# bcgsc/goldrush

Measured on AMD Instinct MI355X. Metric: reads/s through GoldRush-Path (hash + miBF query), higher is better.
Workload: dtype u64

## Files before the change

### goldrush_amd/csrc/grp_batch.inc

```

namespace {

constexpr uint32_t BATCH_MAX_INS = 1u << 17;
constexpr uint32_t BATCH_MAX_BLOCKS = 256;
constexpr uint64_t BATCH_MAX_REC = 1ull << 26;
constexpr unsigned long long BATCH_LOW26 = (1ull << 26) - 1ull;

struct DevBatch
{
  uint32_t epoch = 0;
  uint32_t* bits = nullptr;
  uint64_t cap_mask = 0;
  uint32_t* counters = nullptr;
  uint32_t* chained = nullptr;
  const uint32_t* ins = nullptr;
  uint32_t n_ins = 0, block_tiles = 0;
  uint32_t n_rec = 0;
  unsigned long long* rec_key = nullptr;
  unsigned long long* rec_loc = nullptr;
  unsigned long long* rec_old = nullptr;
  uint32_t* rec_chain = nullptr;
  uint32_t* ovf_next = nullptr;
  uint32_t* ovf_jb = nullptr;
  uint32_t ovf_cap = 0;
// ... 1 lines not shown
  uint32_t* log_head = nullptr;
  uint32_t* log_old = nullptr;
  uint32_t* log_writer = nullptr;
  uint32_t* log_next = nullptr;
  uint32_t* log_slot = nullptr;
  uint64_t log_mask = 0;
  uint32_t log_cap = 0;
  uint32_t first_read = 0;
};

__device__ inline uint32_t
batch_block_id(const DevBatch& b, uint32_t jb)
{
  const uint32_t j = jb >> 8, blk = jb & 255u;
  const uint32_t* e = b.ins + (size_t)j * 6;
  return e[3] + (blk * b.block_tiles + e[4]) / b.block_tiles;
}

__device__ inline uint32_t
wave_counter_take(uint32_t* ctr)
{
  const unsigned long long here = __ballot(1);
  const uint32_t lane = threadIdx.x & 63u;
  const uint32_t leader = (uint32_t)__ffsll((long long)here) - 1u;
  uint32_t base = 0;
  if (lane == leader) {
    base = atomicAdd(ctr, (uint32_t)__popcll(here));
  }
  base = __shfl(base, (int)leader, 64);
  return base + (uint32_t)__popcll(here & ((1ull << lane) - 1ull));
}

__device__ inline uint32_t
batch_unit_jb(const DevBatch& b, uint32_t unit, uint32_t parts)
{
  uint32_t lo = 0, hi = b.n_ins;
  while (hi - lo > 1) {
    const uint32_t mid = (lo + hi) >> 1;
    if (b.ins[(size_t)mid * 6 + 5] <= unit) {
      lo = mid;
    } else {
      hi = mid;
    }
  }
  const uint32_t tj = (unit - b.ins[(size_t)lo * 6 + 5]) / parts;
  return (lo << 8) | (tj / b.block_tiles);
}

template<int H, int WT>
__global__ void __launch_bounds__(THREADS)
k_batch_collect(DevFilter f, DevReads rd, const DevSeeds* __restrict__ sd, uint32_t tile_len, DevBatch b, uint32_t gunit0)
{
  extern __shared__ uint4 smem4[];
  ulonglong2* sTab = reinterpret_cast<ulonglong2*>(smem4);
  const uint32_t hn = frame_seeds<H>(sd);
  uint32_t* sBases = reinterpret_cast<uint32_t*>(sTab + hn * sd->wmax * 4u);

  const uint32_t gunit = gunit0 + blockIdx.x;
  const uint32_t unit = gunit / hn;
  const uint32_t s = gunit - unit * hn;
  const uint32_t parts = gr::geom::tile_parts(frames_per_tile(sd, tile_len));
  const uint32_t jb = batch_unit_jb(b, unit, parts);
  const uint32_t* e = b.ins + (size_t)(jb >> 8) * 6;
  const uint32_t read_idx = e[0], tile_start = e[1];
  const uint32_t u = unit - e[5];
  const uint32_t tj = u / parts, part = u - tj * parts;
  const uint32_t ti = tile_start + tj;
  const uint32_t blk_unit0 = e[5] + (tj / b.block_tiles) * b.block_tiles * parts;
  const uint32_t blk_unit1 = min(blk_unit0 + b.block_tiles * parts, e[5] + (e[2] - e[1]) * parts);
  const uint32_t len = rd.len[read_idx];
  const gr::geom::TileExtent ext = tile_extent(sd, tile_len, len, ti);
  const uint32_t start = ext.start, Lp = ext.Lp, frames = ext.frames;

  load_tab(sTab, sd);
  const uint32_t boff = stage_bases(sBases, rd.packed, rd.word_off[read_idx], len, start, Lp);
  __syncthreads();

  const uint32_t fr = part * THREADS + threadIdx.x;
  const bool live = fr < frames;
  const uint32_t fs = min(min(fr, frames ? frames - 1u : 0u), Lp - sd->span[s]);
  const Probe pr = grp_locate(f, seed_hash_t<WT>(sTab, sd, s, window_at(sBases, boff + fs)));
  uint32_t lr, rel, bit, qid = 0;
  {
    const uint32_t sub = threadIdx.x & 3u, quad_base = (threadIdx.x & 63u) & ~3u;
    const uint4 p0 = f.buckets[quad_bcast64<0>(pr.b) * GRP_UNIT_U4 + sub];
    const uint4 p1 = f.buckets[quad_bcast64<1>(pr.b) * GRP_UNIT_U4 + sub];
    const uint4 p2 = f.buckets[quad_bcast64<2>(pr.b) * GRP_UNIT_U4 + sub];
    const uint4 p3 = f.buckets[quad_bcast64<3>(pr.b) * GRP_UNIT_U4 + sub];
    const QuadAnswer a0 = quad_answer<0>(p0, pr.off, quad_base);
    const QuadAnswer a1 = quad_answer<1>(p1, pr.off, quad_base);
    const QuadAnswer a2 = quad_answer<2>(p2, pr.off, quad_base);
    const QuadAnswer a3 = quad_answer<3>(p3, pr.off, quad_base);
    const QuadAnswer mine = (sub == 0) ? a0 : (sub == 1) ? a1 : (sub == 2) ? a2 : a3;
    lr = mine.lr;
    rel = mine.rel;
    bit = mine.bit;
    qid = mine.id;
  }
  const uint64_t rank = f.super[pr.b >> GRP_SUPER_SHIFT] + rel + lr;
  const bool valid = live && rank < f.pop && bit;
  const uint32_t idx = gunit * THREADS + threadIdx.x;
  const uint64_t home = ((rank + 1) * 0x9E3779B97F4A7C15ULL) >> 20 & b.cap_mask;
  bool claimed = false;
  uint32_t count0 = 0;
  uint32_t* idp = nullptr;
  uint32_t id0 = 0;
  uint32_t why = !live ? 0u : 1u;
  if (valid) {
    unsigned long long* cwp = grp_cw_ptr(f, pr.b, lr, rank);
    idp = (lr < GRP_BUCKET_IDS) ? &reinterpret_cast<uint32_t*>(f.buckets)[grp_id_loc(pr.b, lr)] : nullptr;
    id0 = idp ? qid : 1u;
    unsigned long long cur = (id0 == 0u) ? 0ull : __hip_atomic_load(cwp, __ATOMIC_RELAXED, __HIP_MEMORY_SCOPE_AGENT);
    for (;;) {
      if (grp_claim_epoch(cur) == b.epoch) {
        const uint32_t owner = grp_claim_record(cur);
        const uint32_t owner_unit = owner / (hn * THREADS);
        why = owner + 2u;
        if (owner_unit < blk_unit0 || owner_unit >= blk_unit1) {
          const uint32_t at = wave_counter_take(&b.counters[1]);
          if (at < b.ovf_cap) {
            b.ovf_jb[at] = jb;
            const uint32_t before = atomicExch(&b.rec_chain[owner], at);
            b.ovf_next[at] = before;
            if (before == BATCH_NONE) {
              b.chained[wave_counter_take(&b.counters[0])] = owner;
            }
          }
        }
        break;
      }
      count0 = grp_cnt(cur);
      const unsigned long long prev = atomicCAS(cwp, cur, grp_cnt_with(grp_claim_word(idx, b.epoch, 0u), count0 + 1u));
      if (prev == cur) {
        claimed = true;
        break;
      }
      cur = prev;
    }
  }
  b.rec_key[idx] = claimed ? (((unsigned long long)(rank + 1) << 26) | jb) : (unsigned long long)why;
  if (claimed) {
    const unsigned long long loc = grp_id_loc(pr.b, lr);
    uint32_t* p = idp;
    const uint32_t cur = p ? id0 : grp_ovf_get(f, rank);
    const uint32_t cnt = count0 + 1u;
    const uint32_t id = batch_block_id(b, jb);
    const bool wrote = (uint32_t)(rank ^ (uint64_t)id) % cnt == cnt - 1u;
    if (wrote && cur != 0u) {
      atomicOr(&b.bits[home >> 5], 1u << (home & 31u));
    }
    if (wrote) {
      const uint32_t nv = (cur > 0x80000000u) ? (id | 0x80000000u) : id;
      if (p) {
        *p = nv;
      } else {
        grp_ovf_put(f, rank, nv);
      }
    }
    b.rec_loc[idx] = loc;
    b.rec_old[idx] = ((unsigned long long)(wrote ? 1u : 0u) << 63) | ((unsigned long long)count0 << 32) | cur;
  }
}



__device__ inline uint32_t
batch_next_touch(const DevBatch& b, uint32_t chain, uint32_t own_jb, uint32_t last)
{
  uint32_t best = BATCH_NONE;
  if (last == BATCH_NONE || own_jb > last) {
    best = own_jb;
  }
  for (uint32_t e = chain; e != BATCH_NONE; e = b.ovf_next[e]) {
    const uint32_t jb = b.ovf_jb[e];
    if ((last == BATCH_NONE || jb > last) && jb < best) {
      best = jb;
// ... 689 lines not shown
```

### goldrush_amd/csrc/grp_kernels.inc

```

__device__ inline uint64_t
window_lo(const uint32_t* sBases, uint32_t b)
{
  uint32_t bit = b * 2u;
  uint32_t wi = bit >> 5;
  uint32_t sh = bit & 31u;
  uint64_t lo = (uint64_t)sBases[wi] | ((uint64_t)sBases[wi + 1] << 32);
  uint64_t w = lo >> sh;
  if (sh) {
    w |= (uint64_t)sBases[wi + 2] << (64u - sh);
  }
  return w;
}

struct Win
{
  uint64_t lo;
  const uint32_t* src;
  uint32_t b;
};

__device__ inline Win
window_at(const uint32_t* sBases, uint32_t b)
{
// ... 357 lines not shown
      for (uint32_t q = 1; q < GRP_UNIT_U4; ++q) {
        buckets[b * GRP_UNIT_U4 + q] = make_uint4(0, 0, 0, 0);
      }
    }
    rel += (uint32_t)__popcll(bm[i]);
  }
  ovf = wave_sum(ovf);
  far = wave_sum(far);
  if ((threadIdx.x & 63) == 0 && ovf) {
    atomicAdd(n_ovf, (unsigned long long)ovf);
  }
  if ((threadIdx.x & 63) == 0 && far) {
    atomicAdd(n_ovf + 1, (unsigned long long)far);
  }
}

__global__ void __launch_bounds__(THREADS)
k_far_build(DevFilter f)
{
  for (uint64_t b = (uint64_t)blockIdx.x * THREADS + threadIdx.x; b < f.n_buckets; b += (uint64_t)gridDim.x * THREADS) {
    const uint4 hd = f.buckets[b * GRP_UNIT_U4];
    const uint32_t c = (uint32_t)__popcll(grp_bitmap(hd));
    if (c <= GRP_NEAR_CW) {
      continue;
    }
    const uint64_t base = f.super[b >> GRP_SUPER_SHIFT] + hd.x;
    for (uint32_t lr = GRP_NEAR_CW; lr < c; ++lr) {
      const unsigned long long key = base + lr + 1;
      uint64_t slot = (key * 0x9E3779B97F4A7C15ULL) >> 19 & f.far_mask;
      for (;;) {
        if (f.far[slot].x == 0ull && atomicCAS(&f.far[slot].x, 0ull, key) == 0ull) {
          break;
        }
        slot = (slot + 1) & f.far_mask;
      }
    }
  }
}

__global__ void __launch_bounds__(THREADS)
k_far_reset(ulonglong2* __restrict__ far, uint64_t n)
{
  for (uint64_t i = (uint64_t)blockIdx.x * THREADS + threadIdx.x; i < n; i += (uint64_t)gridDim.x * THREADS) {
    far[i].y = 0ull;
  }
}

__global__ void __launch_bounds__(THREADS)
k_reset_bucket_ids(uint4* __restrict__ buckets, uint64_t n_buckets)
{
  for (uint64_t i = (uint64_t)blockIdx.x * THREADS + threadIdx.x; i < n_buckets * GRP_UNIT_U4; i += (uint64_t)gridDim.x * THREADS) {
    if ((i & (GRP_UNIT_U4 - 1u)) == 0) {
      reinterpret_cast<uint32_t*>(&buckets[i])[3] = 0u;
    } else {
      buckets[i] = make_uint4(0, 0, 0, 0);
    }
  }
}


template<int G>
__device__ inline uint32_t
quad_bcast(uint32_t v)
{
  return (uint32_t)__builtin_amdgcn_mov_dpp((int)v, G * 0x55, 0xF, 0xF, true);
}

template<int G>
__device__ inline uint64_t
quad_bcast64(uint64_t v)
{
  return (uint64_t)quad_bcast<G>((uint32_t)v) | ((uint64_t)quad_bcast<G>((uint32_t)(v >> 32)) << 32);
}

struct QuadAnswer
{
  uint32_t bit;
  uint32_t lr;
  uint32_t id;
  uint32_t rel;
};

template<int G>
__device__ inline QuadAnswer
quad_answer(const uint4& piece, uint32_t off, uint32_t quad_base)
{
  const uint32_t o = quad_bcast<G>(off);
  const uint64_t bm = (uint64_t)quad_bcast<0>(piece.y) | ((uint64_t)quad_bcast<0>(piece.z) << 32);
  QuadAnswer a;
  a.rel = quad_bcast<0>(piece.x);
  a.bit = (uint32_t)((bm >> o) & 1ull);
  a.lr = grp_local_rank(bm, o);
  const uint32_t slot = 3u + min(a.lr, GRP_BUCKET_IDS - 1u);
  const uint32_t comp = slot & 3u;
  const uint32_t word = (comp == 0u) ? piece.x : (comp == 1u) ? piece.y : (comp == 2u) ? piece.z : piece.w;
  a.id = (uint32_t)__builtin_amdgcn_ds_bpermute((int)((quad_base + (slot >> 2)) << 2), (int)word);
  return a;
}


__device__ inline void
hist_add(uint32_t* keys, uint32_t* cnts, uint32_t mask, uint32_t id, uint32_t* sDistinct, uint32_t limit, uint32_t* sOverflow)
{
  if (*reinterpret_cast<volatile uint32_t*>(sDistinct) >= limit) {
    *sOverflow = 1u;
    return;
  }
  uint32_t slot = (id * 2654435761u) & mask;
  for (;;) {
    uint32_t old = atomicCAS(&keys[slot], 0u, id);
    if (old == 0u) {
      atomicAdd(sDistinct, 1u);
    }
    if (old == 0u || old == id) {
      atomicAdd(&cnts[slot], 1u);
      return;
    }
    slot = (slot + 1u) & mask;
  }
}

__device__ inline void
hist_add16(uint32_t* keys, uint32_t* cnt_words, uint32_t cap, uint32_t id, uint32_t* sDistinct, uint32_t limit, uint32_t* sOverflow)
{
  if (*reinterpret_cast<volatile uint32_t*>(sDistinct) >= limit) {
    *sOverflow = 1u;
    return;
  }
  uint32_t slot = __umulhi(id * 2654435761u, cap);
  for (;;) {
    uint32_t old = atomicCAS(&keys[slot], 0u, id);
    if (old == 0u) {
      atomicAdd(sDistinct, 1u);
    }
    if (old == 0u || old == id) {
      atomicAdd(&cnt_words[slot >> 1], 1u << ((slot & 1u) << 4));
      return;
    }
    slot = (slot + 1u == cap) ? 0u : slot + 1u;
  }
}

__device__ inline bool
better(uint32_t c, uint32_t id, uint32_t bc, uint32_t bid)
{
  return (c > bc) || (c == bc && c != 0u && id < bid);
}

template<int WT, bool LEFT, bool RIGHT>
__device__ inline void
seed_halves(const ulonglong2* sTab, const DevSeeds* __restrict__ sd, uint32_t n_left, const Win& win, uint64_t& L, uint64_t& RL, uint64_t& R, uint64_t& RR)
{
  const uint64_t w = win.lo;
  L = RL = R = RR = 0;
  const uint32_t wt = WT > 0 ? (uint32_t)WT : sd->weight[0];
  if (n_left == 8u && wt == 16u) {
    if constexpr (LEFT) {
#pragma unroll
      for (uint32_t i = 0; i < 8u; ++i) {
        const ulonglong2 e = sTab[i * 4u + ((uint32_t)(w >> sd->shift[0][i]) & 3u)];
        L ^= e.x;
        RL ^= e.y;
      }
    }
    if constexpr (RIGHT) {
#pragma unroll
      for (uint32_t i = 8u; i < 16u; ++i) {
        const ulonglong2 e = sTab[i * 4u + ((uint32_t)(w >> sd->shift[0][i]) & 3u)];
        R ^= e.x;
        RR ^= e.y;
      }
    }
    return;
  }
  if constexpr (LEFT) {
    for (uint32_t i = 0; i < n_left; ++i) {
      const ulonglong2 e = sTab[i * 4u + ((uint32_t)(w >> sd->shift[0][i]) & 3u)];
      L ^= e.x;
      RL ^= e.y;
    }
  }
  if constexpr (RIGHT) {
// ... 1593 lines not shown
          }
        }
      }
      sTile = pick;
      if (from_dispenser) {
        nxt = atomicAdd(sc.next_tile, 1u);
      }
      if (pick != STREAM_STOP && sc.ctl != nullptr && blockIdx.x < 32u) {
        stream_relay(sc);
      } else if (pick != STREAM_STOP && blockIdx.x < 32u) {
        if (__hip_atomic_load(sc.abort_host, __ATOMIC_RELAXED, __HIP_MEMORY_SCOPE_SYSTEM)) {
          atomicMin(sc.park, 0u);
          atomicMax(sc.next_tile, STREAM_STOP);
          __hip_atomic_store(sc.abort, 1u, __ATOMIC_RELAXED, __HIP_MEMORY_SCOPE_AGENT);
        }
      }
    }
    if (threadIdx.x == 0 && sc.dbg) {
      stc(&sc.dbg[blockIdx.x], 0x30000000u | (sTile & 0x0FFFFFFFu));
    }
    __syncthreads();
    out_idx = sTile;
    if (out_idx == STREAM_STOP) {
      if (!sc.ctl) {
        return;
      }
      pending_event = 1u;
      continue;
    }
  } else {
    out_idx = tile_idx ? tile_idx[blockIdx.x] : blockIdx.x + blk0;
  }
  const uint64_t t = tile_begin + out_idx;
  const uint32_t r = rd.tile_read[t];
  const uint32_t ti = (uint32_t)(t - rd.tile0[r]);
  if constexpr (VER && !ST) {
    if (bv.skip_read_ins != nullptr && r - bv.first < bv.skip_reads) {
      const uint32_t ji = bv.skip_read_ins[r - bv.first];
      if (ji != 0xFFFFFFFFu && ti >= bv.ins[(size_t)ji * 6 + 1] && ti < bv.ins[(size_t)ji * 6 + 2]) {
        return;
      }
    }
  }
  const uint32_t len = rd.len[r];
  const gr::geom::TileExtent ext = tile_extent(sd, tile_len, len, ti);
  const uint32_t start = ext.start, Lp = ext.Lp, frames = ext.frames;

  const uint32_t boff = stage_bases(sBases, rd.packed, rd.word_off[r], len, start, Lp);
  for (uint32_t i = threadIdx.x; i < hist_cap; i += THREADS) {
    sKeys[i] = 0u;
    if (i < hist_cap / 2u) {
      sCnts[i] = 0u;
    }
  }
  if (threadIdx.x == 0) {
    sListN = 0;
    sListW = 0;
    sDistinct = 0;
    sOverflow = 0;
    if constexpr (ST) {
      sCut = 0u;
      if (sFp != nullptr) {
        if (sc.n_fp > 1u) {
          sBuf ^= 1u;
        }
        sHeldTile[sBuf] = STREAM_REDO_NONE;
      }
    }
  }
  __syncthreads();
  if constexpr (ST) {
    if (threadIdx.x == 0) {
      atomicAdd(sc.executed, (unsigned long long)frames * hn);
    }
  }
  uint32_t* const fp_cur = (ST && sFp != nullptr) ? sFp + sBuf * sc.fp_words : nullptr;

  uint32_t n_hit = 0, n_miss = 0;
  uint32_t last[H];
#pragma unroll
  for (int s = 0; s < H; ++s) {
    last[s] = Lp - sd->span[s];
  }
  const uint32_t sub = threadIdx.x & 3u;
  const uint32_t quad_base = (threadIdx.x & 63u) & ~3u;

  const uint32_t n_left = (H >= 2 && H <= GRP_H_GROUP && WT != GRP_WT_LONG) ? sd->n_left : 0u;
  constexpr uint32_t OV = (uint32_t)H - 1u, USE = 64u - OV;
  static_assert(THREADS == 256, "the helper-lane layout below is written for four waves per workgroup (my_wave == 3 is the last one, FBH = 3 * USE + 64)");
  constexpr uint32_t FBH = gr::geom::helper_pass_frames(H);
  const uint32_t ftile = frames_per_tile(sd, tile_len);
  const bool helper = n_left != 0u && (ftile + FBH * FR - 1u) / (FBH * FR) == (ftile + THREADS * FR - 1u) / (THREADS * FR);
  const uint32_t FB = helper ? FBH : (uint32_t)THREADS;
  const uint32_t my_wave = threadIdx.x >> 6, my_lane = threadIdx.x & 63u;
  const uint32_t my_off = helper ? (my_wave * USE + my_lane) : threadIdx.x;
  const bool my_real = helper ? (my_wave == 3u || my_lane < USE) : true;
  const bool my_tail_wave = helper ? my_wave == 3u : true;
  const uint32_t passes = (frames + FB * FR - 1u) / (FB * FR);
  uint64_t bk[FR][H];
  uint32_t off[FR][H];
  bool live_j[FR];
  auto positions = [&](uint32_t pp, uint64_t (&bk_)[FR][H], uint32_t (&off_)[FR][H], bool (&lv)[FR]) {
  if (n_left != 0u) {
#pragma unroll
    for (int j = 0; j < FR; ++j) {
      const uint32_t fr_raw = (pp * FR + j) * FB + my_off;
      const uint32_t fr = min(fr_raw, frames - 1u);
      lv[j] = my_real && fr_raw < frames;
      uint64_t hL, hRL, hR, hRR;
      seed_halves<WT, true, true>(sTab, sd, n_left, window_at(sBases, boff + fr), hL, hRL, hR, hRR);
      const uint64_t hv0 = (hL ^ hR) + (hRL ^ hRR);
#pragma unroll
      for (int s = 0; s < H; ++s) {
        uint64_t hv = hv0;
        if (s != 0) {
          uint64_t nR = __shfl_down((unsigned long long)hR, (unsigned)s, 64);
          uint64_t nRR = __shfl_down((unsigned long long)hRR, (unsigned)s, 64);
          if (my_tail_wave && my_lane + (uint32_t)s >= 64u) {
            uint64_t a, b;
            seed_halves<WT, false, true>(sTab, sd, n_left, window_at(sBases, boff + min(fr_raw + (uint32_t)s, frames - 1u)), a, b, nR, nRR);
          }
          if (lv[j]) {
            if (fr <= last[s]) {
              hv = (srol_small(hL, (uint32_t)s) ^ nR) + (hRL ^ srol_small(nRR, (uint32_t)s));
            } else {
              hv = seed_hash_t<WT>(sTab, sd, s, window_at(sBases, boff + last[s]));
            }
          }
        }
        const Probe p = grp_locate(f, hv);
        bk_[j][s] = p.b;
        off_[j][s] = p.off;
        if constexpr (ST) {
          if (fp_cur != nullptr) {
            fp_cur[((pp * FR + (uint32_t)j) * (uint32_t)THREADS + threadIdx.x) * (uint32_t)H + (uint32_t)s] = lv[j] ? slot_fp(p.b, p.off) : 0u;
          }
        }
      }
    }
  } else {
#pragma unroll
    for (int j = 0; j < FR; ++j) {
      const uint32_t fr_raw = (pp * FR + j) * THREADS + threadIdx.x;
      const uint32_t fr = min(fr_raw, frames - 1u);
      lv[j] = fr_raw < frames;
#pragma unroll
      for (int s = 0; s < H; ++s) {
        if (!seed_on<H>(s, frame_seeds<H>(sd))) {
          bk_[j][s] = 0;
          off_[j][s] = 0;
          if constexpr (ST) {
            if (fp_cur != nullptr) {
              fp_cur[((pp * FR + (uint32_t)j) * (uint32_t)THREADS + threadIdx.x) * (uint32_t)H + (uint32_t)s] = 0u;
            }
          }
          continue;
        }
        const uint64_t hv = seed_hash_t<WT>(sTab, sd, s, window_at(sBases, boff + min(fr, last[s])));
        const Probe p = grp_locate(f, hv);
        bk_[j][s] = p.b;
        off_[j][s] = p.off;
        if constexpr (ST) {
          if (fp_cur != nullptr) {
            fp_cur[((pp * FR + (uint32_t)j) * (uint32_t)THREADS + threadIdx.x) * (uint32_t)H + (uint32_t)s] = lv[j] ? slot_fp(p.b, p.off) : 0u;
          }
        }
      }
    }
  }
  };
  constexpr bool PIPE = (ST || FR == 1) && H <= GRP_H_GROUP;
  if constexpr (PIPE) {
    if (passes > 0u) {
      positions(0u, bk, off, live_j);
    }
  }
  for (uint32_t pass = 0; pass < passes; ++pass) {
    if constexpr (ST) {
      if (sc.ctl && sFp == nullptr && pass != 0u && __hip_atomic_load(sc.abort, __ATOMIC_RELAXED, __HIP_MEMORY_SCOPE_WORKGROUP) != 0u) {
        if (r - sc.first >= ldc(sc.park)) {
          if ((threadIdx.x & 63u) == 0u) {
            sCut = 1u;
          }
          break;
        }
      }
    }
    if constexpr (H <= GRP_H_GROUP) {
      uint4 piece[FR][H][4];
      if constexpr (!PIPE) {
        positions(pass, bk, off, live_j);
      }
#pragma unroll
      for (int j = 0; j < FR; ++j) {
#pragma unroll
        for (int s = 0; s < H; ++s) {
          piece[j][s][0] = f.buckets[quad_bcast64<0>(bk[j][s]) * GRP_UNIT_U4 + sub];
          piece[j][s][1] = f.buckets[quad_bcast64<1>(bk[j][s]) * GRP_UNIT_U4 + sub];
          piece[j][s][2] = f.buckets[quad_bcast64<2>(bk[j][s]) * GRP_UNIT_U4 + sub];
          piece[j][s][3] = f.buckets[quad_bcast64<3>(bk[j][s]) * GRP_UNIT_U4 + sub];
        }
      }
      uint64_t bk_next[PIPE ? FR : 1][PIPE ? H : 1];
      uint32_t off_next[PIPE ? FR : 1][PIPE ? H : 1];
      bool live_next[PIPE ? FR : 1];
      if constexpr (PIPE) {
        if (pass + 1u < passes) {
          positions(pass + 1u, bk_next, off_next, live_next);
        }
      }
#pragma unroll
      for (int j = 0; j < FR; ++j) {
        const bool live = live_j[j];
        bool all = live;
        uint32_t idv[H];
        uint64_t vrank[VER ? H : 1], vbl[VER ? H : 1];
        bool vneed[VER ? H : 1], vamb[VER ? H : 1];
#pragma unroll
        for (int s = 0; s < H; ++s) {
          QuadAnswer a0 = quad_answer<0>(piece[j][s][0], off[j][s], quad_base);
          QuadAnswer a1 = quad_answer<1>(piece[j][s][1], off[j][s], quad_base);
          QuadAnswer a2 = quad_answer<2>(piece[j][s][2], off[j][s], quad_base);
          QuadAnswer a3 = quad_answer<3>(piece[j][s][3], off[j][s], quad_base);
          const QuadAnswer mine = (sub == 0) ? a0 : (sub == 1) ? a1 : (sub == 2) ? a2 : a3;
          all = all && mine.bit;
          uint32_t d = mine.id;

          if (mine.lr >= GRP_BUCKET_IDS && live) {
            d = grp_ovf_get(f, f.super[bk[j][s] >> GRP_SUPER_SHIFT] + mine.rel + mine.lr);
          }
          if constexpr (VER) {
            const uint32_t fl = bv.floor[r - bv.floor_first];
            const uint32_t floor_id = fl & 0x7FFFFFFFu;
            vrank[s] = f.super[bk[j][s] >> GRP_SUPER_SHIFT] + mine.rel + mine.lr;
            vbl[s] = bk[j][s] * 64ull + mine.lr;
            vneed[s] = live && mine.bit && (d & 0x7FFFFFFFu) >= floor_id;
            vamb[s] = (fl >> 31) != 0u && (d & 0x7FFFFFFFu) == floor_id;
          }
          idv[s] = d;
        }
        if (!all) {
          continue;
        }
        if constexpr (VER) {
          batch_view_multi<H>(bv, vrank, vbl, vneed, vamb, r - bv.first, idv);
        }
        uint32_t ids[H];
#pragma unroll
        for (int s = 0; s < H; ++s) {
          const uint32_t d = idv[s];
          const uint32_t id = (d > 0x80000000u) ? (d & 0x7FFFFFFFu) : d;
          if (id == 0u) {
            ++n_miss;
          } else {
            ++n_hit;
          }
          bool dup = false;
#pragma unroll
          for (int u = 0; u < s; ++u) {
            dup = dup || (ids[u] == id);
          }
          ids[s] = id;
          if (id != 0u && !dup) {
            hist_add16(sKeys, sCnts, hist_cap, id, &sDistinct, distinct_limit, &sOverflow);
          }
        }
      }
      if constexpr (PIPE) {
        if (pass + 1u < passes) {
#pragma unroll
          for (int j = 0; j < FR; ++j) {
            live_j[j] = live_next[j];
#pragma unroll
            for (int s = 0; s < H; ++s) {
              bk[j][s] = bk_next[j][s];
              off[j][s] = off_next[j][s];
            }
          }
        }
      }
    } else {
      static_assert(FR == 1 && !PIPE, "the many-seed form runs one frame per lane and pass");
      constexpr int NG = (H + GRP_H_GROUP - 1) / GRP_H_GROUP;
      positions(pass, bk, off, live_j);
      const bool live = live_j[0];
      bool all = live;
      uint32_t idv[H];
      uint64_t vrank[VER ? H : 1], vbl[VER ? H : 1];
      bool vneed[VER ? H : 1], vamb[VER ? H : 1];
#pragma unroll
      for (int s = 0; s < H; ++s) {
        idv[s] = 0u;
        if constexpr (VER) {
          vrank[s] = 0;
          vbl[s] = 0;
          vneed[s] = false;
          vamb[s] = false;
        }
      }
#pragma unroll
      for (int gi = 0; gi < NG; ++gi) {
        uint4 piece[GRP_H_GROUP][4];
#pragma unroll
        for (int q = 0; q < GRP_H_GROUP; ++q) {
          const int s = gi * GRP_H_GROUP + q;
          if (seed_on<H>(s, hn)) {
            piece[q][0] = f.buckets[quad_bcast64<0>(bk[0][s]) * GRP_UNIT_U4 + sub];
            piece[q][1] = f.buckets[quad_bcast64<1>(bk[0][s]) * GRP_UNIT_U4 + sub];
            piece[q][2] = f.buckets[quad_bcast64<2>(bk[0][s]) * GRP_UNIT_U4 + sub];
            piece[q][3] = f.buckets[quad_bcast64<3>(bk[0][s]) * GRP_UNIT_U4 + sub];
          }
        }
#pragma unroll
        for (int q = 0; q < GRP_H_GROUP; ++q) {
          const int s = gi * GRP_H_GROUP + q;
          if (!seed_on<H>(s, hn)) {
            continue;
          }
          QuadAnswer a0 = quad_answer<0>(piece[q][0], off[0][s], quad_base);
          QuadAnswer a1 = quad_answer<1>(piece[q][1], off[0][s], quad_base);
          QuadAnswer a2 = quad_answer<2>(piece[q][2], off[0][s], quad_base);
          QuadAnswer a3 = quad_answer<3>(piece[q][3], off[0][s], quad_base);
          const QuadAnswer mine = (sub == 0) ? a0 : (sub == 1) ? a1 : (sub == 2) ? a2 : a3;
          all = all && mine.bit;
          uint32_t d = mine.id;
          if (mine.lr >= GRP_BUCKET_IDS && live) {
            d = grp_ovf_get(f, f.super[bk[0][s] >> GRP_SUPER_SHIFT] + mine.rel + mine.lr);
          }
          if constexpr (VER) {
            const uint32_t fl = bv.floor[r - bv.floor_first];
            const uint32_t floor_id = fl & 0x7FFFFFFFu;
            vrank[s] = f.super[bk[0][s] >> GRP_SUPER_SHIFT] + mine.rel + mine.lr;
            vbl[s] = bk[0][s] * 64ull + mine.lr;
            vneed[s] = live && mine.bit && (d & 0x7FFFFFFFu) >= floor_id;
            vamb[s] = (fl >> 31) != 0u && (d & 0x7FFFFFFFu) == floor_id;
          }
          idv[s] = d;
        }
      }
      if (all) {
        if constexpr (VER) {
          batch_view_multi<H>(bv, vrank, vbl, vneed, vamb, r - bv.first, idv);
        }
        uint32_t ids[H];
#pragma unroll
        for (int s = 0; s < H; ++s) {
          if (!seed_on<H>(s, hn)) {
            continue;
          }
          const uint32_t d = idv[s];
          const uint32_t id = (d > 0x80000000u) ? (d & 0x7FFFFFFFu) : d;
          if (id == 0u) {
            ++n_miss;
          } else {
            ++n_hit;
          }
          bool dup = false;
#pragma unroll
          for (int u = 0; u < s; ++u) {
            dup = dup || (ids[u] == id);
          }
          ids[s] = id;
          if (id != 0u && !dup) {
            hist_add16(sKeys, sCnts, hist_cap, id, &sDistinct, distinct_limit, &sOverflow);
          }
        }
      }
    }
  }
  if constexpr (ST) {
    if (sc.ctl && threadIdx.x == 0) {
      ev_next = ldc(sc.ctl + SCT_EV + (blockIdx.x % min(SCT_GROUPS, gridDim.x)) * 32u);
    }
  }
  __syncthreads();

  uint32_t bc = 0, bid = 0, my_n = 0;
  for (uint32_t i = threadIdx.x; i < hist_cap; i += THREADS) {
    uint32_t key = tab_word(&sKeys[i]);
    if (key != 0u) {
      uint32_t c = (tab_word(&sCnts[i >> 1]) >> ((i & 1u) << 4)) & 0xFFFFu;
      if (better(c, key, bc, bid)) {
        bc = c;
        bid = key;
      }
      my_n += c > 2u ? 1u : 0u;
    }
  }
#pragma unroll
  for (int o = 32; o > 0; o >>= 1) {
    uint32_t oc = __shfl_xor(bc, o, 64);
    uint32_t oid = __shfl_xor(bid, o, 64);
    if (better(oc, oid, bc, bid)) {
      bc = oc;
      bid = oid;
    }
  }
  n_hit = wave_sum(n_hit);
  n_miss = wave_sum(n_miss);
  my_n = wave_sum(my_n);
  const uint32_t wave = threadIdx.x >> 6;
  if ((threadIdx.x & 63) == 0) {
    sBest[2 * wave] = bc;
    sBest[2 * wave + 1] = bid;
    sRed[2 * wave] = n_hit;
    sRed[2 * wave + 1] = n_miss;
// ... 514 lines not shown
```

### goldrush_amd/csrc/grp_pshard.inc

```

namespace {

constexpr uint32_t PS_CLEAR = 0xFFFFFFFFu;
constexpr uint32_t PS_MAX_OWNERS = 16;

struct DevPshard
{
  uint32_t n_owners;
  uint64_t per_owner;
  uint64_t owner_magic;
  unsigned long long* bin_fill;
  uint64_t bin_cap;
  unsigned long long* keys;
  uint16_t* tags;
  uint32_t* answers;
  uint2* segs;
};

template<int H, int WT>
__global__ void __launch_bounds__(THREADS)
k_ps_partition(DevFilter f, DevReads rd, const DevSeeds* __restrict__ sd, uint32_t tile_len, uint64_t tile_begin, DevPshard ps)
{
  extern __shared__ uint4 smem4[];
  ulonglong2* sTab = reinterpret_cast<ulonglong2*>(smem4);
  uint32_t* sBases = reinterpret_cast<uint32_t*>(sTab + H * sd->wmax * 4u);
  __shared__ uint32_t sCnt[PS_MAX_OWNERS], sPos[PS_MAX_OWNERS];
  __shared__ unsigned long long sOff[PS_MAX_OWNERS];
  const uint64_t t = tile_begin + blockIdx.x;
  const uint32_t r = rd.tile_read[t];
  const uint32_t ti = (uint32_t)(t - rd.tile0[r]);
  const uint32_t len = rd.len[r];
  const uint32_t k = sd->k;
  const gr::geom::TileExtent ext = gr::geom::tile_extent(tile_len, k, k, len, ti);
  const uint32_t start = ext.start, Lp = ext.Lp, frames = ext.frames;
  load_tab(sTab, sd);
  const uint32_t boff = stage_bases(sBases, rd.packed, rd.word_off[r], len, start, Lp);
  if (threadIdx.x < PS_MAX_OWNERS) {
    sCnt[threadIdx.x] = 0;
    sPos[threadIdx.x] = 0;
  }
  __syncthreads();
  for (int pass = 0; pass < 2; ++pass) {
    for (uint32_t fr = threadIdx.x; fr < frames; fr += THREADS) {
#pragma unroll
      for (int s = 0; s < H; ++s) {
        const uint32_t fs = min(fr, Lp - sd->span[s]);
        const Probe pr = grp_locate(f, seed_hash_t<WT>(sTab, sd, s, window_at(sBases, boff + fs)));
        const uint32_t owner = min((uint32_t)__umul64hi(pr.b, ps.owner_magic), ps.n_owners - 1u);
        if (pass == 0) {
          atomicAdd(&sCnt[owner], 1u);
        } else {
          const unsigned long long at = sOff[owner] + atomicAdd(&sPos[owner], 1u);
          if (at < ps.bin_cap) {
            ps.keys[(size_t)owner * ps.bin_cap + at] = (unsigned long long)pr.b * 64ull + pr.off;
            ps.tags[(size_t)owner * ps.bin_cap + at] = (uint16_t)(fr * (uint32_t)H + (uint32_t)s);
          }
        }
      }
    }
    __syncthreads();
    if (pass == 0) {
      if (threadIdx.x < ps.n_owners) {
        const uint32_t n = sCnt[threadIdx.x];
        const unsigned long long at = n ? atomicAdd(&ps.bin_fill[threadIdx.x], (unsigned long long)n) : 0ull;
        sOff[threadIdx.x] = at;
        ps.segs[(size_t)blockIdx.x * ps.n_owners + threadIdx.x] = make_uint2((uint32_t)at, n);
      }
      __syncthreads();
    }
  }
}

__global__ void __launch_bounds__(THREADS)
k_ps_gather(DevFilter f, const unsigned long long* __restrict__ keys, uint32_t* __restrict__ answers, uint64_t n)
{
  const uint32_t sub = threadIdx.x & 3u, quad_base = (threadIdx.x & 63u) & ~3u;
  for (uint64_t i0 = (uint64_t)blockIdx.x * THREADS; i0 < n; i0 += (uint64_t)gridDim.x * THREADS) {
    const uint64_t i = i0 + threadIdx.x;
    const unsigned long long key = i < n ? keys[i] : 0ull;
    const uint64_t b = key >> 6;
    const uint32_t off = (uint32_t)(key & 63ull);
    const uint4 p0 = f.buckets[quad_bcast64<0>(b) * GRP_UNIT_U4 + sub];
    const uint4 p1 = f.buckets[quad_bcast64<1>(b) * GRP_UNIT_U4 + sub];
    const uint4 p2 = f.buckets[quad_bcast64<2>(b) * GRP_UNIT_U4 + sub];
    const uint4 p3 = f.buckets[quad_bcast64<3>(b) * GRP_UNIT_U4 + sub];
    const QuadAnswer a0 = quad_answer<0>(p0, off, quad_base);
    const QuadAnswer a1 = quad_answer<1>(p1, off, quad_base);
    const QuadAnswer a2 = quad_answer<2>(p2, off, quad_base);
    const QuadAnswer a3 = quad_answer<3>(p3, off, quad_base);
    const QuadAnswer mine = (sub == 0) ? a0 : (sub == 1) ? a1 : (sub == 2) ? a2 : a3;
    uint32_t d = mine.id;
    if (mine.lr >= GRP_BUCKET_IDS && mine.bit) {
      d = grp_ovf_get(f, f.super[b >> GRP_SUPER_SHIFT] + mine.rel + mine.lr);
    }
    if (i < n) {
      answers[i] = mine.bit ? d : PS_CLEAR;
    }
  }
}

template<int H>
__global__ void __launch_bounds__(THREADS)
k_ps_vote(DevReads rd, const DevSeeds* __restrict__ sd, uint32_t tile_len, uint64_t tile_begin, DevPshard ps, uint32_t hist_cap, uint32_t distinct_limit, grp_tile_summary* __restrict__ tiles_out,
          grp_id_count* __restrict__ lists_out, uint64_t lists_cap, unsigned long long* __restrict__ list_ctr)
{
  extern __shared__ uint4 smem4[];
  uint32_t* sKeys = reinterpret_cast<uint32_t*>(smem4);
  uint32_t* sCnts = sKeys + hist_cap;
  uint32_t* sAns = sCnts + hist_cap / 2u;
  __shared__ uint32_t sDistinct, sOverflow, sListN, sListW, sBest[2 * (THREADS / 64)], sRed[2 * (THREADS / 64)], sListOff;
  const uint64_t t = tile_begin + blockIdx.x;
  const uint32_t r = rd.tile_read[t];
  const uint32_t ti = (uint32_t)(t - rd.tile0[r]);
  const uint32_t len = rd.len[r];
  const uint32_t k = sd->k;
  const uint32_t frames = gr::geom::tile_extent(tile_len, k, k, len, ti).frames;
  for (uint32_t i = threadIdx.x; i < hist_cap; i += THREADS) {
    sKeys[i] = 0u;
    if (i < hist_cap / 2u) {
      sCnts[i] = 0u;
    }
  }
  if (threadIdx.x == 0) {
    sDistinct = 0;
    sOverflow = 0;
    sListN = 0;
    sListW = 0;
  }
  for (uint32_t o = 0; o < ps.n_owners; ++o) {
    const uint2 sg = ps.segs[(size_t)blockIdx.x * ps.n_owners + o];
    const size_t base = (size_t)o * ps.bin_cap + sg.x;
    for (uint32_t i = threadIdx.x; i < sg.y; i += THREADS) {
      sAns[ps.tags[base + i]] = ps.answers[base + i];
    }
  }
  __syncthreads();
  uint32_t n_hit = 0, n_miss = 0;
  for (uint32_t fr = threadIdx.x; fr < frames; fr += THREADS) {
    uint32_t idv[H];
    bool all = true;
#pragma unroll
    for (int s = 0; s < H; ++s) {
      idv[s] = sAns[fr * (uint32_t)H + (uint32_t)s];
      all = all && idv[s] != PS_CLEAR;
    }
    if (!all) {
      continue;
    }
    uint32_t ids[H];
#pragma unroll
    for (int s = 0; s < H; ++s) {
      const uint32_t d = idv[s];
      const uint32_t id = (d > 0x80000000u) ? (d & 0x7FFFFFFFu) : d;
      if (id == 0u) {
        ++n_miss;
      } else {
        ++n_hit;
      }
      bool dup = false;
#pragma unroll
      for (int u = 0; u < s; ++u) {
        dup = dup || ids[u] == id;
      }
      ids[s] = id;
      if (id != 0u && !dup) {
        hist_add16(sKeys, sCnts, hist_cap, id, &sDistinct, distinct_limit, &sOverflow);
      }
    }
  }
  __syncthreads();
  uint32_t bc = 0, bid = 0, my_n = 0;
  for (uint32_t i = threadIdx.x; i < hist_cap; i += THREADS) {
    const uint32_t key = sKeys[i];
// ... 320 lines not shown
```

Measured before the change: 470,300.

## Rotate quad bucket piece loads so each lane decodes its own bucket

Changes the cooperative 4-lane bucket fetch so each lane loads pieces in a rotated order (sub - G), which leaves the lane owning its own bucket's header word. Each lane then decodes its answer locally, selecting with v_bfi masks, instead of computing all four quad answers via broadcasts and picking one. The goal is to cut cross-lane permutes and redundant rank and decode work per probe. A constexpr predicate keeps the old straight path for some template configurations, and inline asm plus opaque masks adds complexity and a risk of subtle lane-mapping errors.

```diff
diff --git a/goldrush_amd/csrc/grp_batch.inc b/goldrush_amd/csrc/grp_batch.inc
--- a/goldrush_amd/csrc/grp_batch.inc
+++ b/goldrush_amd/csrc/grp_batch.inc
@@ -107,16 +107,14 @@
   const Probe pr = grp_locate(f, seed_hash_t<WT>(sTab, sd, s, window_at(sBases, boff + fs)));
   uint32_t lr, rel, bit, qid = 0;
   {
-    const uint32_t sub = threadIdx.x & 3u, quad_base = (threadIdx.x & 63u) & ~3u;
-    const uint4 p0 = f.buckets[quad_bcast64<0>(pr.b) * GRP_UNIT_U4 + sub];
-    const uint4 p1 = f.buckets[quad_bcast64<1>(pr.b) * GRP_UNIT_U4 + sub];
-    const uint4 p2 = f.buckets[quad_bcast64<2>(pr.b) * GRP_UNIT_U4 + sub];
-    const uint4 p3 = f.buckets[quad_bcast64<3>(pr.b) * GRP_UNIT_U4 + sub];
-    const QuadAnswer a0 = quad_answer<0>(p0, pr.off, quad_base);
-    const QuadAnswer a1 = quad_answer<1>(p1, pr.off, quad_base);
-    const QuadAnswer a2 = quad_answer<2>(p2, pr.off, quad_base);
-    const QuadAnswer a3 = quad_answer<3>(p3, pr.off, quad_base);
-    const QuadAnswer mine = (sub == 0) ? a0 : (sub == 1) ? a1 : (sub == 2) ? a2 : a3;
+    const QuadLane ql = quad_lane();
+    const uint32_t pbytes = quad_piece_bytes(ql.sub);
+    uint4 pc[4];
+    pc[0] = quad_load<0>(f.buckets, pr.b, pbytes);
+    pc[1] = quad_load<1>(f.buckets, pr.b, pbytes);
+    pc[2] = quad_load<2>(f.buckets, pr.b, pbytes);
+    pc[3] = quad_load<3>(f.buckets, pr.b, pbytes);
+    const QuadAnswer mine = quad_decode(pc, pr.off, ql);
     lr = mine.lr;
     rel = mine.rel;
     bit = mine.bit;
diff --git a/goldrush_amd/csrc/grp_kernels.inc b/goldrush_amd/csrc/grp_kernels.inc
--- a/goldrush_amd/csrc/grp_kernels.inc
+++ b/goldrush_amd/csrc/grp_kernels.inc
@@ -463,6 +463,97 @@
 };
 
 template<int G>
+__device__ inline uint32_t
+quad_piece(uint32_t sub)
+{
+  return (sub - (uint32_t)G) & 3u;
+}
+
+__device__ inline uint32_t
+quad_piece_bytes(uint32_t sub)
+{
+  return (quad_piece<0>(sub) << 4) | (quad_piece<1>(sub) << 12) | (quad_piece<2>(sub) << 20) | (quad_piece<3>(sub) << 28);
+}
+
+template<int G>
+__device__ inline uint4
+quad_load(const uint4* buckets, uint64_t b, uint32_t piece_bytes)
+{
+  uint32_t o;
+  asm volatile("v_bfe_u32 %0, %1, %2, 8" : "=v"(o) : "v"(piece_bytes), "n"(8 * G));
+  return *reinterpret_cast<const uint4*>(reinterpret_cast<const char*>(buckets) + (quad_bcast64<G>(b) * (GRP_UNIT_U4 * 16u) + o));
+}
+
+__device__ inline uint32_t
+bit_select(uint32_t m, uint32_t a, uint32_t b)
+{
+  uint32_t r;
+  asm("v_bfi_b32 %0, %1, %2, %3" : "=v"(r) : "v"(m), "v"(a), "v"(b));
+  return r;
+}
+
+__device__ inline uint32_t
+quad_opaque(uint32_t m)
+{
+  asm("" : "+v"(m));
+  return m;
+}
+
+struct QuadLane
+{
+  uint32_t sub;
+  uint32_t quad_base;
+  uint32_t m0, m1, m2;
+};
+
+__device__ inline QuadLane
+quad_lane()
+{
+  QuadLane q;
+  q.sub = threadIdx.x & 3u;
+  q.quad_base = (threadIdx.x & 63u) & ~3u;
+  q.m0 = quad_opaque(q.sub == 0u ? ~0u : 0u);
+  q.m1 = quad_opaque(q.sub == 1u ? ~0u : 0u);
+  q.m2 = quad_opaque(q.sub == 2u ? ~0u : 0u);
+  return q;
+}
+
+__device__ inline uint32_t
+quad_own(const QuadLane& q, uint32_t v0, uint32_t v1, uint32_t v2, uint32_t v3)
+{
+  return bit_select(q.m0, v0, bit_select(q.m1, v1, bit_select(q.m2, v2, v3)));
+}
+
+template<int G>
+__device__ inline uint32_t
+quad_id_round(const uint4& piece, uint32_t slot, int src)
+{
+  const uint32_t sg = quad_bcast<G>(slot);
+  const uint32_t c0 = quad_opaque((uint32_t)((int32_t)(sg << 31) >> 31));
+  const uint32_t c1 = quad_opaque((uint32_t)((int32_t)(sg << 30) >> 31));
+  const uint32_t word = bit_select(c1, bit_select(c0, piece.w, piece.z), bit_select(c0, piece.y, piece.x));
+  return (uint32_t)__builtin_amdgcn_ds_bpermute(src, (int)word);
+}
+
+__device__ __forceinline__ QuadAnswer
+quad_decode(const uint4 (&pc)[4], uint32_t off, const QuadLane& q)
+{
+  const uint64_t bm = (uint64_t)quad_own(q, pc[0].y, pc[1].y, pc[2].y, pc[3].y) | ((uint64_t)quad_own(q, pc[0].z, pc[1].z, pc[2].z, pc[3].z) << 32);
+  QuadAnswer a;
+  a.rel = quad_own(q, pc[0].x, pc[1].x, pc[2].x, pc[3].x);
+  a.bit = (uint32_t)((bm >> off) & 1ull);
+  a.lr = grp_local_rank(bm, off);
+  const uint32_t slot = 3u + min(a.lr, GRP_BUCKET_IDS - 1u);
+  const int src = (int)((q.quad_base + ((q.sub + (slot >> 2)) & 3u)) << 2);
+  const uint32_t r0 = quad_id_round<0>(pc[0], slot, src);
+  const uint32_t r1 = quad_id_round<1>(pc[1], slot, src);
+  const uint32_t r2 = quad_id_round<2>(pc[2], slot, src);
+  const uint32_t r3 = quad_id_round<3>(pc[3], slot, src);
+  a.id = quad_own(q, r0, r1, r2, r3);
+  return a;
+}
+
+template<int G>
 __device__ inline QuadAnswer
 quad_answer(const uint4& piece, uint32_t off, uint32_t quad_base)
 {
@@ -479,6 +570,55 @@
   return a;
 }
 
+__device__ __forceinline__ QuadAnswer
+quad_answer_straight(const uint4 (&pc)[4], uint32_t off, const QuadLane& q)
+{
+  const QuadAnswer a0 = quad_answer<0>(pc[0], off, q.quad_base);
+  const QuadAnswer a1 = quad_answer<1>(pc[1], off, q.quad_base);
+  const QuadAnswer a2 = quad_answer<2>(pc[2], off, q.quad_base);
+  const QuadAnswer a3 = quad_answer<3>(pc[3], off, q.quad_base);
+  const uint32_t sub = q.sub;
+  QuadAnswer a;
+  a.bit = (sub == 0) ? a0.bit : (sub == 1) ? a1.bit : (sub == 2) ? a2.bit : a3.bit;
+  a.lr = (sub == 0) ? a0.lr : (sub == 1) ? a1.lr : (sub == 2) ? a2.lr : a3.lr;
+  a.id = (sub == 0) ? a0.id : (sub == 1) ? a1.id : (sub == 2) ? a2.id : a3.id;
+  a.rel = (sub == 0) ? a0.rel : (sub == 1) ? a1.rel : (sub == 2) ? a2.rel : a3.rel;
+  return a;
+}
+
+template<bool ROT, int G>
+__device__ __forceinline__ uint4
+quad_read(const uint4* buckets, uint64_t b, const QuadLane& q, uint32_t piece_bytes)
+{
+  if constexpr (ROT) {
+    return quad_load<G>(buckets, b, piece_bytes);
+  } else {
+    return buckets[quad_bcast64<G>(b) * GRP_UNIT_U4 + q.sub];
+  }
+}
+
+template<bool ROT>
+__device__ __forceinline__ QuadAnswer
+quad_result(const uint4 (&pc)[4], uint32_t off, const QuadLane& q)
+{
+  if constexpr (ROT) {
+    return quad_decode(pc, off, q);
+  } else {
+    return quad_answer_straight(pc, off, q);
+  }
+}
+
+template<int H, int FR, int WT, bool ST, bool VER, bool GT>
+constexpr bool
+quad_rotated()
+{
+  if (GT && !ST && FR == 1) {
+    if ((H == 3 && WT == -1 && !VER) || (H == 3 && WT == 0 && VER) || (H == 4 && WT == 0 && !VER) || (H > GRP_H_GROUP && WT == 0 && !VER)) {
+      return false;
+    }
+  }
+  return true;
+}
 
 __device__ inline void
 hist_add(uint32_t* keys, uint32_t* cnts, uint32_t mask, uint32_t id, uint32_t* sDistinct, uint32_t limit, uint32_t* sOverflow)
@@ -2238,8 +2378,9 @@
   for (int s = 0; s < H; ++s) {
     last[s] = Lp - sd->span[s];
   }
-  const uint32_t sub = threadIdx.x & 3u;
-  const uint32_t quad_base = (threadIdx.x & 63u) & ~3u;
+  const QuadLane ql = quad_lane();
+  constexpr bool ROT = quad_rotated<H, FR, WT, ST, VER, GT>();
+  const uint32_t pbytes = quad_piece_bytes(ql.sub);
 
   const uint32_t n_left = (H >= 2 && H <= GRP_H_GROUP && WT != GRP_WT_LONG) ? sd->n_left : 0u;
   constexpr uint32_t OV = (uint32_t)H - 1u, USE = 64u - OV;
@@ -2351,10 +2492,10 @@
       for (int j = 0; j < FR; ++j) {
 #pragma unroll
         for (int s = 0; s < H; ++s) {
-          piece[j][s][0] = f.buckets[quad_bcast64<0>(bk[j][s]) * GRP_UNIT_U4 + sub];
-          piece[j][s][1] = f.buckets[quad_bcast64<1>(bk[j][s]) * GRP_UNIT_U4 + sub];
-          piece[j][s][2] = f.buckets[quad_bcast64<2>(bk[j][s]) * GRP_UNIT_U4 + sub];
-          piece[j][s][3] = f.buckets[quad_bcast64<3>(bk[j][s]) * GRP_UNIT_U4 + sub];
+          piece[j][s][0] = quad_read<ROT, 0>(f.buckets, bk[j][s], ql, pbytes);
+          piece[j][s][1] = quad_read<ROT, 1>(f.buckets, bk[j][s], ql, pbytes);
+          piece[j][s][2] = quad_read<ROT, 2>(f.buckets, bk[j][s], ql, pbytes);
+          piece[j][s][3] = quad_read<ROT, 3>(f.buckets, bk[j][s], ql, pbytes);
         }
       }
       uint64_t bk_next[PIPE ? FR : 1][PIPE ? H : 1];
@@ -2374,11 +2515,7 @@
         bool vneed[VER ? H : 1], vamb[VER ? H : 1];
 #pragma unroll
         for (int s = 0; s < H; ++s) {
-          QuadAnswer a0 = quad_answer<0>(piece[j][s][0], off[j][s], quad_base);
-          QuadAnswer a1 = quad_answer<1>(piece[j][s][1], off[j][s], quad_base);
-          QuadAnswer a2 = quad_answer<2>(piece[j][s][2], off[j][s], quad_base);
-          QuadAnswer a3 = quad_answer<3>(piece[j][s][3], off[j][s], quad_base);
-          const QuadAnswer mine = (sub == 0) ? a0 : (sub == 1) ? a1 : (sub == 2) ? a2 : a3;
+          const QuadAnswer mine = quad_result<ROT>(piece[j][s], off[j][s], ql);
           all = all && mine.bit;
           uint32_t d = mine.id;
 
@@ -2461,10 +2598,10 @@
         for (int q = 0; q < GRP_H_GROUP; ++q) {
           const int s = gi * GRP_H_GROUP + q;
           if (seed_on<H>(s, hn)) {
-            piece[q][0] = f.buckets[quad_bcast64<0>(bk[0][s]) * GRP_UNIT_U4 + sub];
-            piece[q][1] = f.buckets[quad_bcast64<1>(bk[0][s]) * GRP_UNIT_U4 + sub];
-            piece[q][2] = f.buckets[quad_bcast64<2>(bk[0][s]) * GRP_UNIT_U4 + sub];
-            piece[q][3] = f.buckets[quad_bcast64<3>(bk[0][s]) * GRP_UNIT_U4 + sub];
+            piece[q][0] = quad_read<ROT, 0>(f.buckets, bk[0][s], ql, pbytes);
+            piece[q][1] = quad_read<ROT, 1>(f.buckets, bk[0][s], ql, pbytes);
+            piece[q][2] = quad_read<ROT, 2>(f.buckets, bk[0][s], ql, pbytes);
+            piece[q][3] = quad_read<ROT, 3>(f.buckets, bk[0][s], ql, pbytes);
           }
         }
 #pragma unroll
@@ -2473,11 +2610,7 @@
           if (!seed_on<H>(s, hn)) {
             continue;
           }
-          QuadAnswer a0 = quad_answer<0>(piece[q][0], off[0][s], quad_base);
-          QuadAnswer a1 = quad_answer<1>(piece[q][1], off[0][s], quad_base);
-          QuadAnswer a2 = quad_answer<2>(piece[q][2], off[0][s], quad_base);
-          QuadAnswer a3 = quad_answer<3>(piece[q][3], off[0][s], quad_base);
-          const QuadAnswer mine = (sub == 0) ? a0 : (sub == 1) ? a1 : (sub == 2) ? a2 : a3;
+          const QuadAnswer mine = quad_result<ROT>(piece[q], off[0][s], ql);
           all = all && mine.bit;
           uint32_t d = mine.id;
           if (mine.lr >= GRP_BUCKET_IDS && live) {
diff --git a/goldrush_amd/csrc/grp_pshard.inc b/goldrush_amd/csrc/grp_pshard.inc
--- a/goldrush_amd/csrc/grp_pshard.inc
+++ b/goldrush_amd/csrc/grp_pshard.inc
@@ -74,21 +74,19 @@
 __global__ void __launch_bounds__(THREADS)
 k_ps_gather(DevFilter f, const unsigned long long* __restrict__ keys, uint32_t* __restrict__ answers, uint64_t n)
 {
-  const uint32_t sub = threadIdx.x & 3u, quad_base = (threadIdx.x & 63u) & ~3u;
+  const QuadLane ql = quad_lane();
+  const uint32_t pbytes = quad_piece_bytes(ql.sub);
   for (uint64_t i0 = (uint64_t)blockIdx.x * THREADS; i0 < n; i0 += (uint64_t)gridDim.x * THREADS) {
     const uint64_t i = i0 + threadIdx.x;
     const unsigned long long key = i < n ? keys[i] : 0ull;
     const uint64_t b = key >> 6;
     const uint32_t off = (uint32_t)(key & 63ull);
-    const uint4 p0 = f.buckets[quad_bcast64<0>(b) * GRP_UNIT_U4 + sub];
-    const uint4 p1 = f.buckets[quad_bcast64<1>(b) * GRP_UNIT_U4 + sub];
-    const uint4 p2 = f.buckets[quad_bcast64<2>(b) * GRP_UNIT_U4 + sub];
-    const uint4 p3 = f.buckets[quad_bcast64<3>(b) * GRP_UNIT_U4 + sub];
-    const QuadAnswer a0 = quad_answer<0>(p0, off, quad_base);
-    const QuadAnswer a1 = quad_answer<1>(p1, off, quad_base);
-    const QuadAnswer a2 = quad_answer<2>(p2, off, quad_base);
-    const QuadAnswer a3 = quad_answer<3>(p3, off, quad_base);
-    const QuadAnswer mine = (sub == 0) ? a0 : (sub == 1) ? a1 : (sub == 2) ? a2 : a3;
+    uint4 pc[4];
+    pc[0] = quad_load<0>(f.buckets, b, pbytes);
+    pc[1] = quad_load<1>(f.buckets, b, pbytes);
+    pc[2] = quad_load<2>(f.buckets, b, pbytes);
+    pc[3] = quad_load<3>(f.buckets, b, pbytes);
+    const QuadAnswer mine = quad_decode(pc, off, ql);
     uint32_t d = mine.id;
     if (mine.lr >= GRP_BUCKET_IDS && mine.bit) {
       d = grp_ovf_get(f, f.super[b >> GRP_SUPER_SHIFT] + mine.rel + mine.lr);
```

Result: faster. 483,100, median of 6 (+2.7%).
